# mitake/k8s

Measured on AMD Instinct MI355X. Metric: images/sec ResNet-50 TfJob (train, synthetic ImageNet), higher is better.
Workload: dtype bf16; 1 GPU; model=resnet50-v1.5, global_batch=3072, per_gpu_batch=3072, image_size=224, parallelism=dp1, optimizer=fused SGD momentum 0.9 (HIP)

## Files before the change

### k8s_amd/csrc/binding/conv.cpp

```cpp
#include "binding/common.h"

namespace k8s_amd::binding {
namespace {

int conv_out(int in, int k, int st, int pad, int dil) { return (in + 2 * pad - dil * (k - 1) - 1) / st + 1; }

struct ConvGeom {
  int N, H, W, C, K, R, S;
};
ConvGeom conv_geom(const Tensor& x, const Tensor& w) {
  TORCH_CHECK(x.dim() == 4 && w.dim() == 4, "x [N,H,W,C], w [K,R,S,C]");
  ConvGeom g{(int)x.size(0), (int)x.size(1), (int)x.size(2), (int)x.size(3),
             (int)w.size(0), (int)w.size(1), (int)w.size(2)};
  TORCH_CHECK(w.size(3) == g.C, "channel mismatch");
  TORCH_CHECK(g.C % 8 == 0 && g.K % 8 == 0, "implicit-GEMM conv needs C % 8 == 0 and K % 8 == 0");
  return g;
}
Tensor conv_fwd(Tensor x, Tensor w, int64_t stride, int64_t pad, int64_t dil, bool out_f32, OptTensor bias, int64_t act,
                OptTensor stats, OptTensor xform) {
  check_bf16(x, "x"); check_bf16(w, "w");
  const auto [N, H, W, C, K, R, S] = conv_geom(x, w);
  TORCH_CHECK(stride >= 1 && dil >= 1, "conv_fwd: stride >= 1, dilation >= 1");
  const int Ho = conv_out(H, R, stride, pad, dil), Wo = conv_out(W, S, stride, pad, dil);
  if (bias) check_channel_f32(*bias, K, "bias");
  if (stats) check_stat_sums(*stats, K, "stats", true);
  const float* xf = xform_ptr(xform, C);
  if (xf) TORCH_CHECK(C % 64 == 0 && !out_f32 && !bias && act == 0,
                      "normalize-on-load convolution: C % 64 == 0, bf16 output, no bias / activation");
  auto y = torch::empty({N, Ho, Wo, K}, x.options().dtype(out_f32 ? at::kFloat : at::kBFloat16));
  launch_conv_fwd(cbf(x), cbf(w), y.data_ptr(), out_f32, N, H, W, C, K, R, S, (int)stride, (int)pad, (int)dil, Ho, Wo,
                  optf(bias), (int)act, 0, stats ? f32(*stats) : nullptr, cur_stream(), nullptr, xf);
  return y;
}

Tensor conv_infer(Tensor x, Tensor w, int64_t stride, int64_t pad, Tensor scale, Tensor shift, OptTensor res,
                  bool relu, OptTensor out) {
  check_bf16_dense(x, 4, "x"); check_bf16_dense(w, 4, "w");
  const auto [N, H, W, C, K, R, S] = conv_geom(x, w);
  TORCH_CHECK(stride >= 1 && pad >= 0, "conv_infer: stride >= 1, pad >= 0");
  check_channel_f32(scale, K, "scale"); check_channel_f32(shift, K, "shift");
  TORCH_CHECK(H + 2 * pad >= R && W + 2 * pad >= S, "conv_infer: the filter does not fit the padded image");
  const int Ho = conv_out(H, R, stride, pad, 1), Wo = conv_out(W, S, stride, pad, 1);
  TORCH_CHECK((long)N * Ho * Wo < (1L << 31), "conv_infer: fewer than 2^31 output pixels");
  const std::vector<int64_t> oshape{N, Ho, Wo, K};
  if (out) {
    check_bf16_dense(*out, 4, "out");
    TORCH_CHECK(out->sizes().vec() == oshape, "out must be [N, Ho, Wo, K]");
  }
  if (res) {
    check_bf16_dense(*res, 4, "res");
    TORCH_CHECK(res->sizes().vec() == oshape, "res must have the output's shape [N, Ho, Wo, K]");
  }
  Tensor y = out ? *out : torch::empty(oshape, x.options());
  launch_conv_infer(cbf(x), cbf(w), bf(y), N, H, W, C, K, R, S, (int)stride, (int)pad, Ho, Wo, f32(scale), f32(shift),
                    res ? cbf(*res) : nullptr, relu, cur_stream());
  return y;
}

void conv_fwd_subgrid(Tensor x, Tensor w, int64_t pad, int64_t Hs, int64_t Ws, Tensor out, int64_t stride, int64_t a,
                      int64_t b, bool accumulate, OptTensor bn_x, OptTensor bn_mask, OptTensor bn_mean,
                      OptTensor bn_sums, OptTensor bn_gamma, OptTensor bn_beta, OptTensor bn_invstd) {
  check_bf16(x, "x"); check_bf16(w, "w"); check_bf16(out, "out");
  const auto [N, H, W, C, K, R, S] = conv_geom(x, w);
  TORCH_CHECK(out.dim() == 4 && out.size(0) == N && out.size(3) == K, "out shape");
  const int OH = out.size(1), OW = out.size(2);
  TORCH_CHECK(stride >= 1 && a >= 0 && a < stride && b >= 0 && b < stride, "parity out of range");
  TORCH_CHECK(Hs >= 1 && Ws >= 1 && (Hs - 1) * stride + a < OH && (Ws - 1) * stride + b < OW,
              "sub-grid exceeds the output image");
  k8s_amd::SubGrid sg{OH, OW, (int)stride, (int)a, (int)b};
  k8s_amd::BnBwdSums bb;
  if (bn_sums) {
    TORCH_CHECK(bn_x && bn_mean, "bn sums: bn_x and bn_mean");
    TORCH_CHECK(bn_mask ? accumulate : !accumulate,
                "bn sums: bn_mask + accumulate (a correction) or bn_gamma / bn_beta / bn_invstd + a plain store");
    TORCH_CHECK(bn_x->sizes() == out.sizes(), "bn_x: the shape of out");
    bb = bn_bwd_sums(*bn_x, *bn_mean, *bn_sums, bn_mask, bn_gamma, bn_beta, bn_invstd, {}, {}, {});
  }
  launch_conv_fwd(cbf(x), cbf(w), out.data_ptr(), false, N, H, W, C, K, R, S, 1, (int)pad, 1, (int)Hs, (int)Ws, nullptr,
                  0, accumulate ? 1 : 0, nullptr, cur_stream(), &sg, nullptr, bn_sums ? &bb : nullptr);
}

Tensor conv3x3_dgrad_bnstats(Tensor gy, Tensor wt, Tensor x, Tensor gamma, Tensor beta, Tensor mean, Tensor invstd,
                             Tensor sums) {
  check_bf16_dense(gy, 4, "gy"); check_bf16_dense(wt, 4, "wt"); check_bf16_dense(x, 4, "x");
  const int N = (int)gy.size(0), H = (int)gy.size(1), W = (int)gy.size(2), Kc = (int)gy.size(3);
  const int C = (int)wt.size(0);
  TORCH_CHECK(wt.size(1) == 3 && wt.size(2) == 3 && wt.size(3) == Kc, "wt: [C, 3, 3, K]");
  TORCH_CHECK(x.size(0) == N && x.size(1) == H && x.size(2) == W && x.size(3) == C, "x: the shape of dx");
  TORCH_CHECK(k8s_amd::conv3x3_eligible(H, W, Kc, C, 3, 3, 1, 1, 1), "conv3x3_dgrad_bnstats: outside the kernel");
  const k8s_amd::BnBwdSums bb = bn_bwd_sums(x, mean, sums, {}, gamma, beta, invstd, {}, {}, {});
  Tensor dx = torch::empty({N, H, W, C}, gy.options());
  launch_conv3x3(cbf(gy), cbf(wt), bf(dx), nullptr, nullptr, N, H, W, Kc, C, cur_stream(), &bb);
  return dx;
}

void conv_wgrad(Tensor x, Tensor dy, Tensor dw, int64_t stride, int64_t pad, int64_t dil, int64_t splits,
                bool accumulate, OptTensor xform) {
  check_bf16(x, "x"); check_bf16(dy, "dy");
  check_cuda(dw, "dw"); check_dtype(dw, at::kFloat, "dw");
  const auto [N, H, W, C, K, R, S] = conv_geom(x, dw);
  TORCH_CHECK(stride >= 1 && dil >= 1, "conv_wgrad: stride >= 1, dilation >= 1");
  const int Ho = conv_out(H, R, stride, pad, dil), Wo = conv_out(W, S, stride, pad, dil);
  TORCH_CHECK(dy.dim() == 4 && dy.size(0) == N && dy.size(1) == Ho && dy.size(2) == Wo && dy.size(3) == K,
              "dy shape mismatch");
  const float* xf = xform_ptr(xform, C);
  if (dil == 1 && Ho == H && Wo == W && H == W && k8s_amd::wgrad3x3_tiled_ok(C, K, R, S, (int)stride, (int)pad, W)) {
    auto wsp = torch::empty({k8s_amd::wgrad3x3_tiled_workspace(N, H, W, C)}, dw.options());
    launch_wgrad3x3_tiled(cbf(x), cbf(dy), f32(wsp), f32(dw), N, H, W, C, accumulate, cur_stream(), xf);
    return;
  }
  if (!xf && dil == 1 && k8s_amd::wgrad_stream_eligible(N, Ho, Wo, C, K, R, S)) {
    launch_wgrad_stream(cbf(x), cbf(dy), f32(dw), N, H, W, C, K, R, S, (int)stride, (int)pad, Ho, Wo, accumulate,
                        cur_stream());
    return;
  }
  if (xf) TORCH_CHECK(C % 64 == 0, "normalize-on-load weight gradient needs C % 64 == 0");
  int sp = splits <= 0 ? k8s_amd::gemm_choose_splits(K, R * S * C, N * Ho * Wo) : (int)splits;
  Tensor ws;
  if (sp > 1) ws = torch::empty({k8s_amd::gemm_splitk_workspace(K, R * S * C, sp)}, dw.options());
  launch_conv_wgrad(cbf(x), cbf(dy), f32(dw), N, H, W, C, K, R, S, (int)stride, (int)pad, (int)dil, Ho, Wo, sp,
                    accumulate, sp > 1 ? f32(ws) : nullptr, cur_stream(), xf);
}

std::vector<Tensor> conv_dgrad_wsub(Tensor w, std::vector<std::vector<int64_t>> taps) {
  check_bf16(w, "w");
  TORCH_CHECK(w.dim() == 4, "w [K,R,S,C]");
  const int K = w.size(0), R = w.size(1), S = w.size(2), C = w.size(3);
  TORCH_CHECK(!taps.empty() && taps.size() <= 16, "1-16 parities");
  k8s_amd::DgradTaps t{};
  long off = 0;
  std::vector<int64_t> offs;
  for (size_t p = 0; p < taps.size(); ++p) {
    TORCH_CHECK(!taps[p].empty() && taps[p].size() <= 16, "1-16 taps per parity");
    t.n[p] = (int)taps[p].size();
    t.off[p] = off;
    offs.push_back(off);
    for (size_t i = 0; i < taps[p].size(); ++i) {
      TORCH_CHECK(taps[p][i] >= 0 && taps[p][i] < R * S, "tap index out of range");
      t.rs[p][i] = (int)taps[p][i];
    }
    off += (long)C * t.n[p] * K;
    off = (off + 7) / 8 * 8;
  }
  auto out = torch::empty({off}, w.options());
  launch_conv_dgrad_wsub(cbf(w), bf(out), K, R * S, C, t, (int)taps.size(), cur_stream());
  return {out, torch::tensor(offs)};
}
Tensor conv_dgrad_wtrans(Tensor w) {
  check_bf16(w, "w");
  TORCH_CHECK(w.dim() == 4, "w [K,R,S,C]");
  const int K = w.size(0), R = w.size(1), S = w.size(2), C = w.size(3);
  auto w2 = torch::empty({C, R, S, K}, w.options());
  launch_conv_dgrad_wtrans(cbf(w), bf(w2), K, R, S, C, cur_stream());
  return w2;
}

}

void bind_conv(pybind11::module_& m) {
  m.def("conv_fwd", &conv_fwd, "x"_a, "w"_a, "stride"_a, "pad"_a, "dil"_a, "out_f32"_a, "bias"_a, "act"_a, "stats"_a,
        "xform"_a = py::none());
  m.def("conv_infer", &conv_infer, "x"_a, "w"_a, "stride"_a, "pad"_a, "scale"_a, "shift"_a, "res"_a = py::none(),
        "relu"_a = true, "out"_a = py::none());
  m.def("conv3x3_staged_ok", [](int H, int W, int C, int K, int R, int S, int stride, int pad) {
    return k8s_amd::conv3x3_eligible(H, W, C, K, R, S, stride, pad, 1) &&
           k8s_amd::conv3x3_eligible(H, W, K, C, R, S, stride, pad, 1) &&
           k8s_amd::wgrad3x3_tiled_ok(C, K, R, S, stride, pad, W);
  });
  m.def("conv3x3_dgrad_bnstats", &conv3x3_dgrad_bnstats,
        "3x3 stride-1 data gradient with the BatchNorm-backward sums of a relu(BN(x)) input (conv3x3.hip)");
  m.def("conv_fwd_subgrid", &conv_fwd_subgrid, "x"_a, "w"_a, "pad"_a, "Hs"_a, "Ws"_a, "out"_a, "stride"_a, "a"_a, "b"_a,
        "accumulate"_a = false, "bn_x"_a = py::none(), "bn_mask"_a = py::none(), "bn_mean"_a = py::none(),
        "bn_sums"_a = py::none(), "bn_gamma"_a = py::none(), "bn_beta"_a = py::none(), "bn_invstd"_a = py::none());
  m.def("conv_wgrad", &conv_wgrad, "x"_a, "dy"_a, "dw"_a, "stride"_a, "pad"_a, "dil"_a, "splits"_a, "accumulate"_a,
        "xform"_a = py::none());
  m.def("wgrad_stream_eligible", &k8s_amd::wgrad_stream_eligible, "tall-K weight-gradient kernel takes this shape");
  m.def("conv_dgrad_wtrans", &conv_dgrad_wtrans);
  m.def("conv_dgrad_wsub", &conv_dgrad_wsub);
}

}
```

### k8s_amd/csrc/kernels/launchers.h

```cpp
#pragma once
#include <hip/hip_runtime.h>
#include <stdint.h>

#include "rng.h"

namespace k8s_amd {

int planner_cus();
void set_planner_cus(int n);

void launch_sgd(float* p, float* mom, const void* g, bool g_bf16, uint16_t* pbf, long n, const uint8_t* decay_mask, float lr,
                float mu, float wd, float scale, const float* scale_ptr, const float* hyper, bool nesterov,
                bool first_step, hipStream_t st);
void launch_adam(float* p, float* m1, float* m2, const void* g, bool g_bf16, uint16_t* pbf, long n, const uint8_t* decay_mask,
                 float lr, float b1, float b2, float eps, float wd, float scale, const float* scale_ptr,
                 const float* hyper, float bc1, float bc2, bool decoupled, hipStream_t st);
void launch_sumsq(const void* g, bool g_bf16, long n, float* out, hipStream_t st);
void launch_clip_factor(const float* stats, float max_norm, float* factor, hipStream_t st);
void launch_slice_sum(const uint16_t* in, long n, int world, float* out, uint16_t* out_bf, hipStream_t st);
void launch_cast_bf16(const float* in, uint16_t* out, long n, hipStream_t st);

void launch_grad_accumulate(float* acc, const float* g, long n, bool first, hipStream_t st);
void launch_grad_fold(float* g, const float* acc, uint16_t* out_bf, long n, hipStream_t st);

// ... 20 lines not shown
                             uint16_t* y, const float* sums, int nrep, float* save_mean, float* save_invstd,
                             float* run_mean, float* run_var, float* params, long M, int C, float eps, float momentum,
                             bool relu, hipStream_t st, uint8_t* mask = nullptr, uint16_t* ysub = nullptr,
                             int H = 1, int W = 1);
void launch_bn_fwd_from_sums_dual(const uint16_t* x, const float* gamma, const float* beta, const float* sums,
                                  int nrep, float* save_mean, float* save_invstd, float* run_mean, float* run_var,
                                  float* params, const uint16_t* xr, const float* gamma_r, const float* beta_r,
                                  const float* sums_r, int nrep_r, float* save_mean_r, float* save_invstd_r,
                                  float* run_mean_r, float* run_var_r, float* params_r, uint16_t* y, uint8_t* mask,
                                  long M, int C, float eps, float momentum, hipStream_t st);
void launch_bn_bwd_from_sums(const uint16_t* dy, const uint16_t* x, const uint8_t* mask, const float* sums, int nrep,
                             const float* mean, const float* invstd, const float* gamma, const float* beta,
                             uint16_t* dx, uint16_t* dres, float* dgamma, float* dbeta, float* params, long M, int C,
                             hipStream_t st);
void launch_bn_bwd_relu_from_sums(const uint16_t* dy, const uint16_t* x, const float* sums, int nrep,
                                  const float* mean, const float* invstd, const float* gamma, const float* beta,
                                  uint16_t* dx, float* dgamma, float* dbeta, float* params, long M, int C,
                                  hipStream_t st);
void launch_bn_bwd_dual_from_sums(const uint16_t* dy, const uint8_t* mask, const uint16_t* x, const float* sums,
                                  int nrep, const float* mean, const float* invstd, const float* gamma,
                                  const float* beta, uint16_t* dx, float* dgamma, float* dbeta, float* params,
                                  const uint16_t* x2, const float* sums2, const float* mean2, const float* invstd2,
                                  const float* gamma2, const float* beta2, uint16_t* dx2, float* dgamma2,
                                  float* dbeta2, float* params2, long M, int C, hipStream_t st);
void launch_bn_bwd_dual(const uint16_t* dy, const uint8_t* mask, const uint16_t* x, const float* mean,
                        const float* invstd, const float* gamma, const float* beta, uint16_t* dx, float* dgamma,
                        float* dbeta, float* work, float* params, const uint16_t* x2, const float* mean2,
                        const float* invstd2, const float* gamma2, const float* beta2, uint16_t* dx2, float* dgamma2,
                        float* dbeta2, float* work2, float* params2, long M, int C, hipStream_t st);
void launch_bn_finalize_sums(const float* gamma, const float* beta, const float* sums, int nrep, float* save_mean,
                             float* save_invstd, float* run_mean, float* run_var, float* params, long M, int C,
                             float eps, float momentum, hipStream_t st);
constexpr int kConvStatReplicas = 32;
void launch_bn_bwd(const uint16_t* dy, const uint16_t* x, const float* mean, const float* invstd, const float* gamma,
                   const float* beta, bool relu_x, uint16_t* dx, uint16_t* dres, float* dgamma, float* dbeta,
                   float* work, float* params, long M, int C, hipStream_t st, const uint8_t* mask = nullptr);
void launch_relu_mask(const uint16_t* y, uint8_t* mask, long nvec, hipStream_t st);

void launch_norm_fwd(bool rms, const uint16_t* x, const uint16_t* res, uint16_t* xsum, const float* gamma,
                     const float* beta, uint16_t* y, float* mean, float* rstd, long R, int D, float eps,
                     hipStream_t st, const DropArgs* drop = nullptr);
int norm_workspace_floats(long R, int D);
void launch_norm_bwd(bool rms, const uint16_t* dy, const uint16_t* x, const float* gamma, const float* mean,
                     const float* rstd, const uint16_t* dres, uint16_t* dx, float* dgamma, float* dbeta, float* work,
                     long R, int D, hipStream_t st, float* dsum = nullptr, const DropArgs* drop = nullptr,
                     uint16_t* da = nullptr);

void launch_dropout(const uint16_t* x, uint16_t* y, long R, int D, const DropArgs& dr, hipStream_t st);
void launch_dropout_mask(uint8_t* out, long row0, long R, int C, const DropArgs& dr, hipStream_t st);

void launch_xent_fwd(const void* logits, bool bf16, const int64_t* labels, long R, long V, long ld, float* loss,
                     float* lse, long ignore_index, float smoothing, hipStream_t st);
void launch_xent_bwd(const void* logits, bool bf16, const int64_t* labels, const float* lse, const float* dscale,
                     bool per_row, long R, long V, long ld, void* dlogits, long ignore_index, float smoothing,
                     hipStream_t st);
void launch_xent_eval(const void* logits, bool bf16, const int64_t* labels, long R, long V, long ld, float* loss,
                      int* rank, long ignore_index, hipStream_t st);

int gemm_choose_splits(int M, int N, int K);
struct AddEpi {
  const uint16_t* src;
  const uint8_t* mask;
};
bool gemm_short_ok(int M, int N, int K, long lda, long ldc);
bool gemm_short_bnstats_ok(int M, int N, int K, bool dual);
struct BnBwdSums {
  const uint16_t* x = nullptr;
  const float* gamma = nullptr;
  const float* beta = nullptr;
  const float* mean = nullptr;
  const float* invstd = nullptr;
  float* sums = nullptr;
  const uint8_t* mask = nullptr;
  const uint16_t* x2 = nullptr;
  const float* mean2 = nullptr;
  float* sums2 = nullptr;
};
struct GemmShortBnStats {
  const uint16_t* x = nullptr;
  const uint8_t* mask = nullptr;
  const float* mean = nullptr;
  float* sums = nullptr;
  const uint16_t* x2 = nullptr;
  const float* mean2 = nullptr;
  float* sums2 = nullptr;
};
void launch_gemm_short(const uint16_t* A, const uint16_t* B, long ldb, bool b_mn, uint16_t* C, const uint16_t* add,
                       const uint8_t* mask, const float* xf, float* stats, int M, int N, int K, int epi,
                       hipStream_t st, const GemmShortBnStats* bst = nullptr);
void launch_gemm_dgrad_bnstats(const uint16_t* A, const uint16_t* B, uint16_t* C, int M, int N, int K,
                               const BnBwdSums& bb, hipStream_t st, bool accumulate = false,
                               const uint16_t* add_src = nullptr, const uint8_t* add_mask = nullptr);
void launch_gemm(const uint16_t* A, long lda, bool a_kmajor, const uint16_t* B, long ldb, bool b_kmajor, void* C,
                 long ldc, bool c_f32, int M, int N, int K, const float* bias, int act, uint16_t* pre, int mode,
                 float alpha, int splits, float* ws, hipStream_t st, const AddEpi* add = nullptr,
                 const float* xform_b = nullptr, int xform_c = 0);
void launch_mask_apply(const uint16_t* src, const uint8_t* mask, uint16_t* out, long n, hipStream_t st);
long gemm_splitk_workspace(int M, int N, int splits);
bool conv3x3_eligible(int H, int W, int C, int K, int R, int S, int stride, int pad, int dil);
void launch_conv3x3(const uint16_t* x, const uint16_t* w, uint16_t* y, float* stats, const float* xform, int N,
                    int H, int W, int C, int K, hipStream_t st,
                    const BnBwdSums* bsums = nullptr);
bool gemm256_eligible(int M, int N, int K, bool a_kmajor, bool b_kmajor);
int gemm256_choose_splits(int M, int N, int K);
bool gemm_w4_dact_ok(int M, int N, int K, long lda, long ldb, long ldc);
long gemm_w4_dact_part_floats(int M, int N);
void launch_gemm_w4_dact(const uint16_t* A, long lda, const uint16_t* B, long ldb, uint16_t* C, long ldc, int M, int N,
                         int K, const uint16_t* pre, int act, float* part, float* db, bool db_accumulate,
                         float* sk_slabs, int* sk_sync, hipStream_t st);
bool gemm_w4_swiglu_ok(int M, int F, int K, long lda, long ldb);
void launch_gemm_w4_swiglu_bwd(const uint16_t* A, long lda, const uint16_t* B, long ldb, uint16_t* dgu,
                               const uint16_t* gu, int M, int F, int K, int blk, float* sk_slabs, int* sk_sync,
                               hipStream_t st);
bool gemm_w4_stats_ok(int M, int N, int K);
bool gemm_w4_dgrad_bnstats_ok(int M, int N, int K);
void launch_gemm_w4_dgrad_bnstats(const uint16_t* A, const uint16_t* B, uint16_t* y, int M, int N, int K,
                                  const uint16_t* x, const float* tab, float* sums, float* sk_slabs, int* sk_sync,
                                  hipStream_t st);
void launch_gemm_w4_stats(const uint16_t* A, long lda, const uint16_t* B, long ldb, uint16_t* y, int M, int N, int K,
                          float* stats, float* sk_slabs, int* sk_sync, hipStream_t st);
bool gemm_w4_rope_ok(int M, int N, int K, long lda, long ldb, int rot_cols);
void launch_gemm_w4_rope(const uint16_t* A, long lda, const uint16_t* B, long ldb, uint16_t* y, int M, int N, int K,
                         const int* pos, const float* table, int rot_cols, float* sk_slabs, int* sk_sync,
                         hipStream_t st);
bool gemm_w4_swiglu_fwd_ok(int M, int F, int K, long lda, long ldb);
void launch_gemm_w4_swiglu_fwd(const uint16_t* A, long lda, const uint16_t* B, long ldb, uint16_t* gu, uint16_t* h,
                               int M, int F, int K, float* sk_slabs, int* sk_sync, hipStream_t st);
struct Gemm256Plan {
  int tiles, full, sk, kps;
};
Gemm256Plan gemm256_plan(int M, int N, int K);
long gemm256_sk_slab_floats(const Gemm256Plan& p);
long gemm256_sk_sync_ints(const Gemm256Plan& p);
void launch_gemm256(const uint16_t* A, long lda, bool a_kmajor, const uint16_t* B, long ldb, bool b_kmajor, void* C,
                    long ldc, bool c_f32, int M, int N, int K, const float* bias, int act, uint16_t* pre,
                    bool accumulate, float alpha, hipStream_t st, int splits = 1, float* ws = nullptr,
                    float* sk_slabs = nullptr, int* sk_sync = nullptr);
struct SubGrid {
  int H, W, stride, a, b;
};
void launch_conv_fwd(const uint16_t* x, const uint16_t* w, void* y, bool y_f32, int N, int H, int W, int C, int K,
                     int R, int S, int stride, int pad, int dil, int Ho, int Wo, const float* bias, int act,
                     int mode, float* stats, hipStream_t st, const SubGrid* sg = nullptr, const float* xform = nullptr,
                     const BnBwdSums* bb = nullptr);
void launch_conv_infer(const uint16_t* x, const uint16_t* w, uint16_t* y, int N, int H, int W, int C, int K, int R,
                       int S, int stride, int pad, int Ho, int Wo, const float* scale, const float* shift,
                       const uint16_t* res, bool relu, hipStream_t st);
void launch_conv_wgrad(const uint16_t* x, const uint16_t* dy, float* dw, int N, int H, int W, int C, int K, int R,
                       int S, int stride, int pad, int dil, int Ho, int Wo, int splits, bool accumulate, float* ws,
                       hipStream_t st, const float* xform = nullptr);
bool wgrad_stream_eligible(int N, int Ho, int Wo, int C, int K, int R, int S);
void launch_wgrad_stream(const uint16_t* x, const uint16_t* dy, float* dw, int N, int H, int W, int C, int K, int R,
                         int S, int stride, int pad, int Ho, int Wo, bool accumulate, hipStream_t st);
void launch_conv_dgrad_wtrans(const uint16_t* w, uint16_t* w2, int K, int R, int S, int C, hipStream_t st);
struct DgradTaps {
  int n[16];
  long off[16];
  int rs[16][16];
};
void launch_conv_dgrad_wsub(const uint16_t* w, uint16_t* out, int K, int RS, int C, const DgradTaps& taps, int np,
                            hipStream_t st);

void launch_swiglu_fwd(const uint16_t* gu, uint16_t* y, long T, int F, int blk, hipStream_t st);
void launch_swiglu_bwd(const uint16_t* gu, const uint16_t* dy, uint16_t* dgu, long T, int F, int blk, hipStream_t st);
void launch_rope(uint16_t* x, long ld, const int* pos, const float* table, long T, int H, int D, bool inverse,
                 hipStream_t st);
void launch_gelu_bwd(const uint16_t* dy, const uint16_t* pre, uint16_t* dx, long n, hipStream_t st);
void launch_relu_bwd(const uint16_t* dy, const uint16_t* y, uint16_t* dx, long n, hipStream_t st);
int colsum_workspace_floats(long R, int C);
void launch_colsum(const uint16_t* x, long R, int C, float* work, float* out, bool accumulate, hipStream_t st);
void launch_colsum_fold(float* part, int P, int C, float* out, bool accumulate, hipStream_t st);
void launch_colsum_group(float* part, int P, int C, int gs, hipStream_t st);
void launch_act_bwd_colsum(int act, const uint16_t* dy, const uint16_t* pre, uint16_t* g, long R, int C, float* work,
                           float* out, bool accumulate, hipStream_t st);

struct AttnFwdArgs {
  const uint16_t *q, *k, *v;
  uint16_t* o;
  float* lse;
  const int* kv_lens;
  long sqb, sqs, sqh, skb, sks, skh, svb, svs, svh, sob, sos, soh;
  long lse_ld;
  int B, Sq, Sk, Hq, Hkv, causal;
  float scale_log2;
  DropArgs drop;
};
struct AttnBwdArgs {
  const uint16_t *q, *k, *v, *dO;
  const float* lse;
  float* delta;
  uint16_t* dq;
  uint16_t *dk, *dv;
  const int* kv_lens;
  long sqb, sqs, sqh, skb, sks, skh, svb, svs, svh, sdb, sds, sdh;
  long sgqb, sgqs, sgqh, sgkb, sgks, sgkh, sgvb, sgvs, sgvh;
  long lse_ld;
  int B, Sq, Sk, Hq, Hkv, causal;
  float scale_log2, scale;
  int dkv_split = 1;
  float* dkv_ws = nullptr;
  float* cpart = nullptr;
  int cpart_ld = 0;
  DropArgs drop;
};
int flash_dkv_splits(int B, int Sq, int Sk, int Hkv, int causal);
bool flash_bwd_one_block(int D, int Sq, int Sk, int Hq, int Hkv, int dkv_split);
void launch_bn_relu_maxpool_fwd(const uint16_t* x, const float* gamma, const float* beta, const float* sums, int nrep,
                                float* save_mean, float* save_invstd, float* run_mean, float* run_var, float* params,
                                uint16_t* y, uint8_t* idx, int N, int H, int W, int C, float eps, float momentum,
                                hipStream_t st, uint16_t* xarg = nullptr, uint8_t* ybits = nullptr);
void launch_pool_bn_bwd_from_sums(const uint16_t* dpool, const uint8_t* idx, const uint16_t* x, const float* mean,
                                  const float* invstd, const float* gamma, const float* beta, uint16_t* dx,
                                  float* dgamma, float* dbeta, const float* sums, int nrep, float* params, int N,
                                  int H, int W, int C, hipStream_t st);
int pool_bn_workspace_floats(int C);
void launch_pool_bn_bwd(const uint16_t* dpool, const uint8_t* idx, const uint16_t* x, const float* mean,
                        const float* invstd, const float* gamma, const float* beta, uint16_t* dx, float* dgamma,
                        float* dbeta, float* work, float* params, int N, int H, int W, int C, hipStream_t st);

int stream_order_mode();
int stream_dir(int fixed);

void launch_flash_fwd(const AttnFwdArgs& a, int D, hipStream_t st);
void launch_flash_bwd(const AttnBwdArgs& a, int D, const uint16_t* o, long sob, long sos, long soh, hipStream_t st);

struct EmbTable {
  const uint16_t* w;
  float* g;
  const int64_t* ids;
  int V;
};
void launch_embed_fwd(const EmbTable* tabs, int ntab, int T, int D, int S, uint16_t* out, hipStream_t st);
void launch_embed_bwd(const EmbTable* tabs, int ntab, int T, int D, int S, const uint16_t* g, hipStream_t st);

void launch_avgpool_fwd(const uint16_t* x, uint16_t* y, int N, int HW, int C, hipStream_t st);
void launch_avgpool_bwd(const uint16_t* dy, uint16_t* dx, int N, int HW, int C, hipStream_t st);

void launch_stem_s2d_input(const uint16_t* x, int N, int H, int W, int Cin, int pad, uint16_t* out, hipStream_t st);
void launch_stem_w_s2d(const uint16_t* w7, int K, int R, int Cw, uint16_t* w4, hipStream_t st);
bool stem_conv_fwd_ok(int K, int R, int C, int Wo);
void launch_stem_conv_fwd(const uint16_t* xs, const uint16_t* w4, uint16_t* y, float* stats, int N, int Hs, int Ws,
                          hipStream_t st);
void splitk_reduce(const float* ws, int splits, long mn, float* out, bool accumulate, hipStream_t st);
bool wgrad3x3_tiled_ok(int C, int K, int R, int S, int stride, int pad, int W);
int wgrad3x3_tiled_blocks(int N, int H, int W, int C);
long wgrad3x3_tiled_workspace(int N, int H, int W, int C);
void launch_wgrad3x3_tiled(const uint16_t* x, const uint16_t* dy, float* ws, float* dw, int N, int H, int W, int C,
                           bool accumulate, hipStream_t st, const float* xform = nullptr);
int stem_wgrad_blocks(int N, int Hs);
void launch_stem_wgrad(const uint16_t* xs, const uint16_t* dy, float* ws, float* dw4, int N, int Hs, int Ws,
                       hipStream_t st);
void launch_stem_dw_s2d(const float* dw4, int K, int R, int Cw, float* dw7, hipStream_t st);

void launch_subsample_nhwc(const uint16_t* x, uint16_t* y, int N, int H, int W, int C, int s, hipStream_t st);
void launch_maxpool_fwd(const uint16_t* x, uint16_t* y, uint8_t* idx, int N, int H, int W, int C, int Ho, int Wo,
                        int k, int s, int p, hipStream_t st);
void launch_maxpool_bwd(const uint16_t* dy, const uint8_t* idx, uint16_t* dx, int N, int H, int W, int C, int Ho,
                        int Wo, int k, int s, int p, hipStream_t st);

}
```

### k8s_amd/ops/conv.py

```python
from __future__ import annotations

import os
import warnings

import torch
import torch.nn.functional as F

from k8s_amd.ops._ext import load as _load



STATS = {"hip_fwd": 0, "aten_fwd": 0, "hip_wgrad": 0, "aten_wgrad": 0, "hip_dgrad": 0, "aten_dgrad": 0,
         "bn_bstats": 0, "hip_infer": 0, "aten_infer": 0}



def _nchw(x):
    return x.permute(0, 3, 1, 2)


def _nhwc(y):
    return y.permute(0, 2, 3, 1).contiguous()


# ... 80 lines not shown
BSTATS_STRIDED = os.environ.get("K8S_AMD_BN_BSTATS_STRIDED", "0") != "0"
BSTATS_TILE_SHORT = os.environ.get("K8S_AMD_BN_BSTATS_TILE_SHORT", "0") != "0"


def _bn_sums(C_, bn_link, C, device):
    R = C_.conv_stat_replicas
    if bn_link.store is not None:
        from k8s_amd.ops.nn import _zero_scratch
        return _zero_scratch(bn_link.store, device, R * 2 * C).view(R, 2, C)
    return torch.zeros(R, 2, C, device=device, dtype=torch.float32)


def _dgrad_hip(C_, gy, w, padding, addend=None, bn_link=None):
    K, R, S, C = w.shape
    masked = addend is not None and not torch.is_tensor(addend)
    if (BSTATS_3X3 and bn_link is not None and bn_link.relu and bn_link.x is not None and addend is None and R == 3
            and S == 3
            and padding == 1 and gy.shape[1] == gy.shape[2] and bn_link.x.shape[:3] == gy.shape[:3]
            and C_.conv3x3_staged_ok(gy.shape[1], gy.shape[2], C, K, 3, 3, 1, 1)):
        sums = _bn_sums(C_, bn_link, C, gy.device)
        dx = C_.conv3x3_dgrad_bnstats(gy, C_.conv_dgrad_wtrans(w), bn_link.x, bn_link.gamma, bn_link.beta,
                                      bn_link.mean, bn_link.invstd, sums)
        bn_link.deposit(sums, None, dx)
        return dx
    if R == 1 and S == 1 and padding == 0:
        N, H, W_, _ = gy.shape
        if masked and bn_link is not None and not bn_link.relu and bn_link.x is not None and \
                bn_link.x.shape == (N, H, W_, C) and \
                C_.gemm_short_bnstats_ok(N * H * W_, C, K, bn_link.x2 is not None):
            sums = _bn_sums(C_, bn_link, C, gy.device)
            sums2 = _bn_sums(C_, bn_link, C, gy.device) if bn_link.x2 is not None else None
            out = C_.dgrad_short_bnstats(
                gy.reshape(-1, K), w.reshape(K, C), addend.dy.view(-1, C), addend.mask, bn_link.x.view(-1, C),
                bn_link.mask, bn_link.mean, sums, None if sums2 is None else bn_link.x2.view(-1, C), bn_link.mean2,
                sums2).view(N, H, W_, C)
            bn_link.deposit(sums, sums2, out)
            return out
        if (masked and BSTATS_TILE_MASK and bn_link is not None and not bn_link.relu and bn_link.x is not None
                and bn_link.mask is not None and bn_link.x.shape == (N, H, W_, C) and N * H * W_ < 2 ** 31
                and (BSTATS_TILE_SHORT or bn_link.x2 is None or not C_.gemm_short_bnstats_ok(N * H * W_, C, K, False))):
            out = torch.empty(N, H, W_, C, device=gy.device, dtype=gy.dtype)
            sums = _bn_sums(C_, bn_link, C, gy.device)
            dual = bn_link.x2 is not None
            sums2 = _bn_sums(C_, bn_link, C, gy.device) if dual else None
            C_.gemm_dgrad_bnstats_mask(gy.reshape(-1, K), w.reshape(K, C), out.view(-1, C), bn_link.x.view(-1, C),
                                       bn_link.mask, bn_link.mean, sums, addend.dy.view(-1, C), addend.mask,
                                       bn_link.x2.view(-1, C) if dual else None, bn_link.mean2 if dual else None,
                                       sums2)
            bn_link.deposit(sums, sums2, out)
            return out
        if (BSTATS_GEMM and bn_link is not None and bn_link.relu and bn_link.x is not None and addend is None
                and bn_link.x.shape == (N, H, W_, C) and C_.gemm_dgrad_bnstats_ok(N * H * W_, C, K)):
            sums = _bn_sums(C_, bn_link, C, gy.device)
            out = C_.gemm_dgrad_bnstats(gy.reshape(-1, K), w.reshape(K, C), bn_link.x.view(-1, C), bn_link.gamma,
                                        bn_link.beta, bn_link.mean, bn_link.invstd, sums).view(N, H, W_, C)
            bn_link.deposit(sums, None, out)
            return out
        if (BSTATS_ENTRY and addend is None and bn_link is not None and not bn_link.relu and not bn_link.last_full and bn_link.mask is not None
                and bn_link.x2 is None and bn_link.x is not None and bn_link.x.shape == (N, H, W_, C)
                and C_.gemm_short_bnstats_ok(N * H * W_, C, K, False)):
            sums = _bn_sums(C_, bn_link, C, gy.device)
            out = C_.dgrad_short_bnstats(gy.reshape(-1, K), w.reshape(K, C), None, None, bn_link.x.view(-1, C),
                                         bn_link.mask, bn_link.mean, sums).view(N, H, W_, C)
            bn_link.deposit_pending(sums)
            return out
        if masked:
            out = torch.empty(N, H, W_, C, device=gy.device, dtype=gy.dtype)
            C_.gemm(gy.reshape(-1, K), True, w.reshape(K, C), False, out.view(-1, C), False, None, 0, None, True,
                    1.0, 1, add_src=addend.dy.view(-1, C), add_mask=addend.mask)
            return out
        if (addend is not None and bn_link is not None and bn_link.last_full and bn_link.x is not None
                and bn_link.mask is not None and bn_link.x.shape == (N, H, W_, C) and addend.is_contiguous()
                and C % 8 == 0 and N * H * W_ < 2 ** 31):
            sums = _bn_sums(C_, bn_link, C, gy.device)
            C_.gemm_dgrad_bnstats_mask(gy.reshape(-1, K), w.reshape(K, C), addend.view(-1, C), bn_link.x.view(-1, C),
                                       bn_link.mask, bn_link.mean, sums)
            bn_link.deposit(sums, None, addend)
            return addend
        if addend is not None:
            C_.gemm(gy.reshape(-1, K), True, w.reshape(K, C), False, addend.view(-1, C), False, None, 0, None, True,
                    1.0, 1)
            return addend
        return C_.gemm(gy.reshape(-1, K), True, w.reshape(K, C), False, None, False, None, 0, None, False, 1.0,
                       1).reshape(N, H, W_, C)
    if masked:
        addend = addend.materialize()
    dx = C_.conv_fwd(gy, C_.conv_dgrad_wtrans(w), 1, R - 1 - padding, 1, False, None, 0, None)
    return dx if addend is None else dx.add_(addend)


def _parity_taps(R, a, pad, stride):
    taps = sorted(((a + pad - r) // stride, r) for r in range(R) if (a + pad - r) % stride == 0)
    if taps and [d for d, _ in taps] != list(range(taps[0][0], taps[0][0] + len(taps))):
        return None
    return taps


def strided_dgrad_ok(gy, w, stride, padding):
    K, R, S, C = w.shape
    if stride < 2 or K % 8 or C % 8:
        return False
    for a in range(stride):
        for b in range(stride):
            tr, ts = _parity_taps(R, a, padding, stride), _parity_taps(S, b, padding, stride)
            if tr is None or ts is None:
                return False
            if tr and ts and tr[0][0] != ts[0][0]:
                return False
    return True


def _dgrad_strided_hip(C_, gy, w, stride, padding, H, W, addend=None, bn_link=None):
    K, R, S, C = w.shape
    N = gy.shape[0]
    fix = (bn_link is not None and bn_link.pending and R == 1 and S == 1 and padding == 0 and addend is not None
           and torch.is_tensor(addend) and addend.is_contiguous() and bn_link.x is not None
           and bn_link.x.shape == addend.shape)
    if bn_link is not None and bn_link.pending and not fix:
        bn_link.sums, bn_link.pending = None, False
    relu_sums = (BSTATS_STRIDED and bn_link is not None and bn_link.relu and bn_link.x is not None and addend is None
                 and not bn_link.pending and bn_link.x.shape == (N, H, W, C) and C > 64 and K % 64 == 0)
    rsums = _bn_sums(C_, bn_link, C, gy.device) if relu_sums else None
    parities = [(a, b) for a in range(stride) for b in range(stride)]
    empty = [(a, b) for a, b in parities
             if not _parity_taps(R, a, padding, stride) or not _parity_taps(S, b, padding, stride)]
    if addend is not None:
        dx = addend
    else:
        dx = (torch.zeros if empty else torch.empty)(N, H, W, C, device=gy.device, dtype=gy.dtype)
    live = [(a, b, _parity_taps(R, a, padding, stride), _parity_taps(S, b, padding, stride))
            for a in range(stride) for b in range(stride)]
    live = [(a, b, tr, ts) for a, b, tr, ts in live if tr and ts]
    packed, offs = C_.conv_dgrad_wsub(w, [[r * S + s_ for _, r in tr for _, s_ in ts] for _, _, tr, ts in live])
    offs = offs.tolist()
    for i, (a, b, tr, ts) in enumerate(live):
        n = C * len(tr) * len(ts) * K
        wsub = packed[offs[i]:offs[i] + n].view(C, len(tr), len(ts), K)
        Hs, Ws = (H - a + stride - 1) // stride, (W - b + stride - 1) // stride
        if fix:
            C_.conv_fwd_subgrid(gy, wsub, -tr[0][0], Hs, Ws, dx, stride, a, b, True, bn_link.x, bn_link.mask,
                                bn_link.mean, bn_link.sums)
        elif relu_sums:
            C_.conv_fwd_subgrid(gy, wsub, -tr[0][0], Hs, Ws, dx, stride, a, b, False, bn_link.x, None, bn_link.mean,
                                rsums, bn_link.gamma, bn_link.beta, bn_link.invstd)
        else:
            C_.conv_fwd_subgrid(gy, wsub, -tr[0][0], Hs, Ws, dx, stride, a, b, addend is not None)
    if fix:
        bn_link.complete(dx)
    if relu_sums:
        bn_link.deposit(rsums, None, dx)
    return dx


def conv_bwd(gy, x, w, stride, padding, need_dx, p=None, addend=None, xform=None, x_sub=None, bn_link=None):
    K, R, S, C = w.shape
    C_ = _load() if gy.is_cuda else None
    if x_sub is not None:
        _wgrad_hip(C_, gy, x_sub, p.grad.view(p.shape), 1, 0, p.written)
        STATS["hip_wgrad"] += 1
        p.store._notify(p) if p.written else p.store.mark_written(p)
        p = None
    hip = _hip(gy, x, w)
    if xform is not None and not (hip and C % 64 == 0 and K % 8 == 0 and p is not None
                                  and p.grad.dtype == torch.float32):
        raise RuntimeError("normalize-on-load weight gradient outside the kernels' contract")
    if addend is not None and not torch.is_tensor(addend) and not (
            hip and stride == 1 and K % 8 == 0 and C % 8 == 0):
        addend = addend.materialize()
    dw_done = False
    if hip and C % 8 == 0 and K % 8 == 0 and p is not None and p.grad.dtype == torch.float32:
        STATS["hip_wgrad"] += 1
        acc = p.written
        _wgrad_hip(C_, gy, x, p.grad.view(p.shape), stride, padding, acc, xform)
        if acc:
            p.store._notify(p)
        else:
            p.store.mark_written(p)
        dw_done = True
    dx = None
    if need_dx:
        if hip and stride == 1 and K % 8 == 0 and C % 8 == 0:
            STATS["hip_dgrad"] += 1
            dx = _dgrad_hip(C_, gy, w, padding, addend, bn_link)
        elif hip and strided_dgrad_ok(gy, w, stride, padding):
            STATS["hip_dgrad"] += 1
            dx = _dgrad_strided_hip(C_, gy, w, stride, padding, x.shape[1], x.shape[2], addend, bn_link)
        else:
            _vendor("dgrad", x, w, stride, padding)
            dx, _ = _aten_bwd(gy, x, w, stride, padding, True, False)
            if addend is not None:
                dx = dx + addend
    return _finish_dw(dx, dw_done, p, gy, x, w, stride, padding)


SUB1X1 = os.environ.get("K8S_AMD_SUB1X1", "1") != "0"


def subsample_ok(x, w, stride, padding) -> bool:
    K, R, S, C = w.shape
    return (SUB1X1 and stride > 1 and R == 1 and S == 1 and padding == 0 and _hip(x, w) and C % 64 == 0
            and K % 8 == 0 and x.is_contiguous())


def _finish_dw(dx, dw_done, p, gy, x, w, stride, padding):
    if not dw_done and p is not None:
        _vendor("wgrad", x, w, stride, padding)
        _, dw = _aten_bwd(gy, x, w, stride, padding, False, True)
        p.store.deposit(p, dw)
    return dx
```

Baseline: 15680 images/s.

## Fuse 1x1 conv backward dgrad, wgrad and BatchNorm-backward sums into one kernel

Adds a HIP kernel for the bottleneck 1x1 expansion convs (C,K = 64,256 or 128,512). In one persistent pass over row tiles it computes the data gradient with MFMA and writes it out. It also applies the BN normalize-on-load to x to build the weight gradient, and accumulates the BN-backward sums for the upstream relu(BN) input. This avoids reading gy and x several times across separate dgrad, wgrad and stats kernels. The cost is heavy register and LDS use at one block per CU, plus atomic dw and sums reductions. The path is on by default behind an env flag.

```diff
diff --git a/k8s_amd/csrc/binding/conv.cpp b/k8s_amd/csrc/binding/conv.cpp
--- a/k8s_amd/csrc/binding/conv.cpp
+++ b/k8s_amd/csrc/binding/conv.cpp
@@ -92,6 +92,23 @@
   Tensor dx = torch::empty({N, H, W, C}, gy.options());
   launch_conv3x3(cbf(gy), cbf(wt), bf(dx), nullptr, nullptr, N, H, W, Kc, C, cur_stream(), &bb);
   return dx;
+}
+
+Tensor bwd1x1_fused(Tensor gy, Tensor x, Tensor w, Tensor xform, Tensor gamma, Tensor beta, Tensor mean, Tensor invstd,
+                    Tensor dw, Tensor sums, bool accumulate) {
+  check_bf16_dense(gy, 2, "gy"); check_bf16_dense(x, 2, "x"); check_bf16_dense(w, 2, "w");
+  const long M = gy.size(0), K = gy.size(1), C = x.size(1);
+  TORCH_CHECK(x.size(0) == M && w.size(0) == K && w.size(1) == C, "shapes: gy [M, K], x [M, C], w [K, C]");
+  TORCH_CHECK(k8s_amd::bwd1x1_fused_ok(M, (int)C, (int)K),
+              "bwd1x1_fused: (C, K) = (64, 256) or (128, 512), 1 <= M < 2^31");
+  check_cuda(dw, "dw"); check_dtype(dw, at::kFloat, "dw"); check_aligned(dw, "dw");
+  TORCH_CHECK(dw.numel() == K * C, "dw must have K * C fp32 elements");
+  check_channel_f32(xform, 2 * C, "xform (BatchNorm scale | shift)");
+  const k8s_amd::BnBwdSums bb = bn_bwd_sums(x, mean, sums, {}, gamma, beta, invstd, {}, {}, {});
+  Tensor dz = torch::empty({M, C}, gy.options());
+  launch_bwd1x1_fused(cbf(gy), cbf(x), cbf(w), f32(xform), bb.gamma, bb.beta, bb.mean, bb.invstd, bf(dz), f32(dw),
+                      bb.sums, M, (int)C, (int)K, accumulate, cur_stream());
+  return dz;
 }
 
 void conv_wgrad(Tensor x, Tensor dy, Tensor dw, int64_t stride, int64_t pad, int64_t dil, int64_t splits,
@@ -174,7 +191,13 @@
         "bn_sums"_a = py::none(), "bn_gamma"_a = py::none(), "bn_beta"_a = py::none(), "bn_invstd"_a = py::none());
   m.def("conv_wgrad", &conv_wgrad, "x"_a, "dy"_a, "dw"_a, "stride"_a, "pad"_a, "dil"_a, "splits"_a, "accumulate"_a,
         "xform"_a = py::none());
-  m.def("wgrad_stream_eligible", &k8s_amd::wgrad_stream_eligible, "tall-K weight-gradient kernel takes this shape");
+  m.def("bwd1x1_fused", &bwd1x1_fused, "gy"_a, "x"_a, "w"_a, "xform"_a, "gamma"_a, "beta"_a, "mean"_a, "invstd"_a,
+        "dw"_a, "sums"_a, "accumulate"_a,
+        "1x1 data gradient, normalize-on-load weight gradient and BatchNorm-backward sums in one pass (bwd1x1_fused.hip)");
+  m.def("bwd1x1_fused_ok", [](int64_t M, int64_t C, int64_t K) {
+    return C <= 1024 && K <= 4096 && k8s_amd::bwd1x1_fused_ok(M, (int)C, (int)K);
+  }, "M"_a, "C"_a, "K"_a, "whether bwd1x1_fused takes this shape");
+  m.def("wgrad_stream_eligible",&k8s_amd::wgrad_stream_eligible, "tall-K weight-gradient kernel takes this shape");
   m.def("conv_dgrad_wtrans", &conv_dgrad_wtrans);
   m.def("conv_dgrad_wsub", &conv_dgrad_wsub);
 }
diff --git a/k8s_amd/csrc/kernels/bwd1x1_fused.hip b/k8s_amd/csrc/kernels/bwd1x1_fused.hip
--- /dev/null
+++ b/k8s_amd/csrc/kernels/bwd1x1_fused.hip
@@ -0,0 +1,309 @@
+#include <algorithm>
+#include <stdexcept>
+
+#include "common.h"
+#include "launchers.h"
+#include "mfma.h"
+
+namespace k8s_amd {
+namespace b1f {
+
+constexpr int THREADS = 512;
+constexpr int CT = 64;
+
+__device__ __attribute__((aligned(64))) uint16_t g_zero16[64];
+
+typedef __attribute__((ext_vector_type(4))) int int4_t;
+
+__device__ __forceinline__ int swz128(int r) { return 2 * (((r >> 1) & 1) | (((r >> 3) & 1) << 1)); }
+__device__ __forceinline__ int swz_g(int r) { return (2 * ((r & 3) | (((r >> 3) & 1) << 2))) | ((r >> 2) & 1); }
+
+struct TrRaw {
+  short4_t lo, hi;
+};
+template <int RB, bool G>
+__device__ __forceinline__ void tr_load(TrRaw& r, const char* img, int rb, int kk, int lane) {
+  const int g = lane >> 4, i = lane & 15, q = i >> 2, p = i & 3;
+  const int u = (rb >> 3) + (p >> 1);
+  const int r0 = kk * 32 + 8 * g + q, r1 = r0 + 4;
+  const int u0 = u ^ (G ? swz_g(r0) : swz128(r0)), u1 = u ^ (G ? swz_g(r1) : swz128(r1));
+  tr16_asm(r.lo, img + r0 * RB + (u0 << 4) + (p & 1) * 8);
+  tr16_asm(r.hi, img + r1 * RB + (u1 << 4) + (p & 1) * 8);
+}
+#define K8S_LDS_TIE4(w, a, b, c, d) asm volatile(w : "+v"(a), "+v"(b), "+v"(c), "+v"(d))
+
+struct Args {
+  const uint16_t *gy, *x, *w;
+  const float *xform, *gamma, *beta, *mean, *invstd;
+  uint16_t* dz;
+  float* dw;
+  float* sums;
+  int M, C, ntiles, npairs;
+};
+
+__device__ __forceinline__ void lds_barrier() {
+  asm volatile("s_waitcnt lgkmcnt(0)" ::: "memory");
+  __builtin_amdgcn_s_barrier();
+  asm volatile("" ::: "memory");
+}
+
+template <int K, int RS, int NSLOT, int HALVES>
+__global__ void __launch_bounds__(THREADS, 1) bwd1x1_fused_kernel(Args a) {
+  constexpr int RB = K * 2, UG = K / 8;
+  constexpr int IMG_G = RS * RB, IMG_X = RS * 128, STAGE = IMG_G + IMG_X, RING = NSLOT * STAGE;
+  constexpr int LG = RS * UG / THREADS;
+  constexpr int XT = RS * 8;
+  constexpr int NKS = K / 32, KW = K / 8, KTW = KW / 16;
+  static_assert(LG * THREADS == RS * UG && XT % 64 == 0 && XT <= THREADS && (RS == 32 || RS == 64), "tile");
+  static_assert(XT * 64 <= RING, "sums partials reuse the ring");
+  constexpr bool PLDS = K > 256;
+  __shared__ __attribute__((aligned(1024))) char smem[RING + IMG_X + (PLDS ? 5 * CT * 4 : 0)];
+  char* stg = smem + RING;
+  float* ptab = reinterpret_cast<float*>(stg + IMG_X);
+
+  const int tid = threadIdx.x, lane = tid & 63;
+  const int wid = __builtin_amdgcn_readfirstlane(tid >> 6);
+  const int bid = blockIdx.x;
+  int pair = bid, chalf = 0;
+  if constexpr (HALVES == 2) {
+    const int slot = bid >> 3;
+    chalf = slot & 1;
+    pair = (slot >> 1) * 8 + (bid & 7);
+  }
+  const int c0 = chalf * CT;
+  const int n = pair < a.ntiles ? (a.ntiles - pair + a.npairs - 1) / a.npairs : 0;
+  if (n == 0) return;
+  const long M = a.M;
+  const int C = a.C;
+
+  const int ct = wid & 3, rh = wid >> 2;
+  int4_t wf[NKS];
+  {
+    const uint16_t* wp = a.w + (long)(8 * (lane >> 4)) * C + c0 + ct * 16 + (lane & 15);
+#pragma unroll
+    for (int ks = 0; ks < NKS; ++ks) {
+      bf16x8_t v;
+#pragma unroll
+      for (int j = 0; j < 8; ++j) v[j] = (short)wp[(long)(ks * 32 + j) * C];
+      wf[ks] = __builtin_bit_cast(int4_t, v);
+    }
+  }
+  const int erow = tid >> 3;
+  const int eu = (tid & 7) ^ swz128(erow);
+  const int ecol = c0 + eu * 8;
+  float xsc[8], xsh[8], gsc[8], gsh[8], mu[8], ps[8], pq[8];
+#pragma unroll
+  for (int j = 0; j < 8; ++j) {
+    xsc[j] = a.xform[ecol + j];
+    xsh[j] = a.xform[C + ecol + j];
+    mu[j] = a.mean[ecol + j];
+    bn_affine_regs(a.gamma[ecol + j], a.beta[ecol + j], mu[j], a.invstd[ecol + j], gsc[j], gsh[j]);
+    ps[j] = pq[j] = 0.f;
+  }
+  if constexpr (PLDS) {
+    if (tid < 8) {
+#pragma unroll
+      for (int j = 0; j < 8; ++j) {
+        ptab[0 * CT + tid * 8 + j] = xsc[j];
+        ptab[1 * CT + tid * 8 + j] = xsh[j];
+        ptab[2 * CT + tid * 8 + j] = gsc[j];
+        ptab[3 * CT + tid * 8 + j] = gsh[j];
+        ptab[4 * CT + tid * 8 + j] = mu[j];
+      }
+    }
+  }
+#pragma unroll
+  for (int ks = 0; ks < NKS; ++ks) asm volatile("" : "+v"(wf[ks]));
+  if constexpr (!PLDS) {
+#pragma unroll
+    for (int j = 0; j < 8; ++j) asm volatile("" : "+v"(xsc[j]), "+v"(xsh[j]), "+v"(gsc[j]), "+v"(gsh[j]), "+v"(mu[j]));
+  } else {
+    __syncthreads();
+  }
+
+  auto issue = [&](int slot, int i) {
+    char* st = smem + slot * STAGE;
+    const long m0 = (long)(pair + i * a.npairs) * RS;
+#pragma unroll
+    for (int j = 0; j < LG; ++j) {
+      const int sl = j * THREADS + tid, row = sl / UG, up = sl % UG;
+      const int u = up ^ swz_g(row);
+      const long m = m0 + row;
+      const void* src = m < M ? (const void*)(a.gy + m * K + u * 8) : (const void*)g_zero16;
+      glds16(src, st + j * (THREADS * 16) + wid * 1024);
+    }
+    if (wid < XT / 64) {
+      const long m = m0 + erow;
+      const void* src = m < M ? (const void*)(a.x + m * C + ecol) : (const void*)g_zero16;
+      glds16(src, st + IMG_G + wid * 1024);
+    }
+  };
+
+  f32x4_t dwa[KTW][4];
+#pragma unroll
+  for (int i = 0; i < KTW; ++i)
+#pragma unroll
+    for (int j = 0; j < 4; ++j) dwa[i][j] = f32x4_t{0.f, 0.f, 0.f, 0.f};
+
+  const int pre = min(n, NSLOT - 1);
+  for (int s = 0; s < pre; ++s) issue(s, s);
+  int slot = 0;
+  for (int s = 0; s < n; ++s) {
+    const int younger = min(n - 1, s + NSLOT - 2) - s;
+    if (younger >= 2) asm volatile("s_waitcnt vmcnt(%0)" ::"n"(2 * LG) : "memory");
+    else if (younger == 1) asm volatile("s_waitcnt vmcnt(%0)" ::"n"(LG) : "memory");
+    else asm volatile("s_waitcnt vmcnt(0)" ::: "memory");
+    lds_barrier();
+    if (s + NSLOT - 1 < n) issue(slot == 0 ? NSLOT - 1 : slot - 1, s + NSLOT - 1);
+    char* G = smem + slot * STAGE;
+    char* X = G + IMG_G;
+
+    {
+      f32x4_t d0 = {0.f, 0.f, 0.f, 0.f}, d1 = {0.f, 0.f, 0.f, 0.f};
+      const int row0 = rh * (RS / 2) + (lane & 15);
+      const int kq = lane >> 4;
+      if constexpr (RS == 64) {
+        const int row1 = row0 + 16;
+        const char* p0 = G + row0 * RB;
+        const char* p1 = G + row1 * RB;
+        const int s0 = swz_g(row0), s1 = swz_g(row1);
+#pragma unroll
+        for (int ks = 0; ks < NKS; ++ks) {
+          const bf16x8_t b0 = *reinterpret_cast<const bf16x8_t*>(p0 + (((ks * 4 + kq) ^ s0) << 4));
+          const bf16x8_t b1 = *reinterpret_cast<const bf16x8_t*>(p1 + (((ks * 4 + kq) ^ s1) << 4));
+          const mfma_bf16x8 wa = __builtin_bit_cast(mfma_bf16x8, wf[ks]);
+          d0 = mfma16(wa, __builtin_bit_cast(mfma_bf16x8, b0), d0);
+          d1 = mfma16(wa, __builtin_bit_cast(mfma_bf16x8, b1), d1);
+        }
+      } else {
+        const char* p0 = G + row0 * RB;
+        const int s0 = swz_g(row0);
+#pragma unroll
+        for (int ks = 0; ks < NKS; ks += 2) {
+          const bf16x8_t b0 = *reinterpret_cast<const bf16x8_t*>(p0 + (((ks * 4 + kq) ^ s0) << 4));
+          const bf16x8_t b1 = *reinterpret_cast<const bf16x8_t*>(p0 + (((ks * 4 + 4 + kq) ^ s0) << 4));
+          d0 = mfma16(__builtin_bit_cast(mfma_bf16x8, wf[ks]), __builtin_bit_cast(mfma_bf16x8, b0), d0);
+          d1 = mfma16(__builtin_bit_cast(mfma_bf16x8, wf[ks + 1]), __builtin_bit_cast(mfma_bf16x8, b1), d1);
+        }
+        d0 += d1;
+      }
+      const int unit = ct * 2 + (lane >> 5), half = (lane >> 4) & 1;
+      auto put = [&](int row, const f32x4_t& d) {
+        bf16x4_t o;
+#pragma unroll
+        for (int r = 0; r < 4; ++r) o[r] = (short)f2bf(d[r]);
+        *reinterpret_cast<bf16x4_t*>(stg + row * 128 + ((unit ^ swz128(row)) << 4) + half * 8) = o;
+      };
+      put(row0, d0);
+      if constexpr (RS == 64) put(row0 + 16, d1);
+    }
+    lds_barrier();
+
+    if (wid < XT / 64) {
+      const bf16x8_t dzv = *reinterpret_cast<const bf16x8_t*>(stg + tid * 16);
+      const bf16x8_t xv = *reinterpret_cast<const bf16x8_t*>(X + tid * 16);
+      if constexpr (PLDS) {
+        const float* t = ptab + (ecol - c0);
+#pragma unroll
+        for (int j = 0; j < 8; ++j) {
+          xsc[j] = t[j];
+          xsh[j] = t[CT + j];
+          gsc[j] = t[2 * CT + j];
+          gsh[j] = t[3 * CT + j];
+          mu[j] = t[4 * CT + j];
+        }
+      }
+      float o[8];
+#pragma unroll
+      for (int j = 0; j < 8; ++j) {
+        const float xf = bf2f((uint16_t)xv[j]);
+        o[j] = fmaxf(__builtin_fmaf(xf, xsc[j], xsh[j]), 0.f);
+        const float g = relu_on(xf, gsc[j], gsh[j]) ? bf2f((uint16_t)dzv[j]) : 0.f;
+        ps[j] += g;
+        pq[j] = __builtin_fmaf(g, xf - mu[j], pq[j]);
+      }
+      *reinterpret_cast<bf16x8_t*>(X + tid * 16) = pack_bf16x8(o);
+      const long m = (long)(pair + s * a.npairs) * RS + erow;
+      if (m < M) *reinterpret_cast<bf16x8_t*>(a.dz + m * C + ecol) = dzv;
+    }
+    lds_barrier();
+
+#pragma unroll
+    for (int kk = 0; kk < RS / 32; ++kk) {
+      TrRaw ar[KTW], br[4];
+#pragma unroll
+      for (int j = 0; j < 4; ++j) tr_load<128, false>(br[j], X, j * 16, kk, lane);
+#pragma unroll
+      for (int i = 0; i < KTW; ++i) tr_load<RB, true>(ar[i], G, wid * KW + i * 16, kk, lane);
+      K8S_LDS_TIE8("s_waitcnt lgkmcnt(0)", br[0].lo, br[0].hi, br[1].lo, br[1].hi, br[2].lo, br[2].hi, br[3].lo,
+                   br[3].hi);
+#pragma unroll
+      for (int i = 0; i < KTW; i += 2)
+        K8S_LDS_TIE4("s_waitcnt lgkmcnt(0)", ar[i].lo, ar[i].hi, ar[i + 1].lo, ar[i + 1].hi);
+#pragma unroll
+      for (int i = 0; i < KTW; ++i)
+#pragma unroll
+        for (int j = 0; j < 4; ++j)
+          dwa[i][j] = __builtin_amdgcn_mfma_f32_16x16x32_bf16(join8(br[j].lo, br[j].hi), join8(ar[i].lo, ar[i].hi),
+                                                              dwa[i][j], 0, 0, 0);
+    }
+    slot = slot + 1 == NSLOT ? 0 : slot + 1;
+  }
+
+#pragma unroll
+  for (int i = 0; i < KTW; ++i) {
+    const int k = wid * KW + i * 16 + (lane & 15);
+#pragma unroll
+    for (int j = 0; j < 4; ++j) {
+      float* d = a.dw + (long)k * C + c0 + j * 16 + 4 * (lane >> 4);
+#pragma unroll
+      for (int r = 0; r < 4; ++r) atomicAdd(d + r, dwa[i][j][r]);
+    }
+  }
+  __syncthreads();
+  float* part = reinterpret_cast<float*>(smem);
+  if (tid < XT) {
+#pragma unroll
+    for (int j = 0; j < 8; ++j) {
+      part[tid * 16 + j] = ps[j];
+      part[tid * 16 + 8 + j] = pq[j];
+    }
+  }
+  __syncthreads();
+  if (tid < 2 * CT) {
+    const int col = tid & (CT - 1), which = tid / CT;
+    const int u = col >> 3, r = col & 7;
+    float v = 0.f;
+#pragma unroll 4
+    for (int row = 0; row < RS; ++row) v += part[(row * 8 + (u ^ swz128(row))) * 16 + which * 8 + r];
+    atomicAdd(a.sums + (long)(bid % kConvStatReplicas) * 2 * C + (long)which * C + c0 + col, v);
+  }
+}
+
+}
+
+bool bwd1x1_fused_ok(long M, int C, int K) {
+  return M >= 1 && M < (1L << 31) && ((C == 64 && K == 256) || (C == 128 && K == 512));
+}
+
+void launch_bwd1x1_fused(const uint16_t* gy, const uint16_t* x, const uint16_t* w, const float* xform,
+                         const float* gamma, const float* beta, const float* mean, const float* invstd, uint16_t* dz,
+                         float* dw, float* sums, long M, int C, int K, bool accumulate, hipStream_t st) {
+  using namespace b1f;
+  if (!bwd1x1_fused_ok(M, C, K)) throw std::runtime_error("bwd1x1_fused: (C, K) = (64, 256) or (128, 512), M < 2^31");
+  if (!accumulate) (void)hipMemsetAsync(dw, 0, (size_t)K * C * sizeof(float), st);
+  Args a{gy, x, w, xform, gamma, beta, mean, invstd, dz, dw, sums, (int)M, C, 0, 0};
+  const int cus = std::max(1, planner_cus());
+  if (C == 64) {
+    a.ntiles = (int)((M + 63) / 64);
+    a.npairs = cus;
+    hipLaunchKernelGGL((bwd1x1_fused_kernel<256, 64, 3, 1>), dim3(cus), dim3(THREADS), 0, st, a);
+  } else {
+    const int grid = std::max(16, cus / 16 * 16);
+    a.ntiles = (int)((M + 31) / 32);
+    a.npairs = grid / 2;
+    hipLaunchKernelGGL((bwd1x1_fused_kernel<512, 32, 4, 2>), dim3(grid), dim3(THREADS), 0, st, a);
+  }
+}
+
+}
diff --git a/k8s_amd/csrc/kernels/launchers.h b/k8s_amd/csrc/kernels/launchers.h
--- a/k8s_amd/csrc/kernels/launchers.h
+++ b/k8s_amd/csrc/kernels/launchers.h
@@ -196,6 +196,10 @@
 bool wgrad_stream_eligible(int N, int Ho, int Wo, int C, int K, int R, int S);
 void launch_wgrad_stream(const uint16_t* x, const uint16_t* dy, float* dw, int N, int H, int W, int C, int K, int R,
                          int S, int stride, int pad, int Ho, int Wo, bool accumulate, hipStream_t st);
+bool bwd1x1_fused_ok(long M, int C, int K);
+void launch_bwd1x1_fused(const uint16_t* gy, const uint16_t* x, const uint16_t* w, const float* xform,
+                         const float* gamma, const float* beta, const float* mean, const float* invstd, uint16_t* dz,
+                         float* dw, float* sums, long M, int C, int K, bool accumulate, hipStream_t st);
 void launch_conv_dgrad_wtrans(const uint16_t* w, uint16_t* w2, int K, int R, int S, int C, hipStream_t st);
 struct DgradTaps {
   int n[16];
diff --git a/k8s_amd/ops/conv.py b/k8s_amd/ops/conv.py
--- a/k8s_amd/ops/conv.py
+++ b/k8s_amd/ops/conv.py
@@ -256,6 +256,16 @@
     return dx
 
 
+def _bwd1x1_fused_on() -> bool:
+    return os.environ.get("K8S_AMD_BWD1X1_FUSED", "1") != "0"
+
+
+def _fused_link_ok(bn_link, x) -> bool:
+    return (bn_link is not None and bn_link.relu and bn_link.x is not None and bn_link.x.shape == x.shape
+            and bn_link.x.data_ptr() == x.data_ptr()
+            and all(t is not None for t in (bn_link.gamma, bn_link.beta, bn_link.mean, bn_link.invstd)))
+
+
 def conv_bwd(gy, x, w, stride, padding, need_dx, p=None, addend=None, xform=None, x_sub=None, bn_link=None):
     K, R, S, C = w.shape
     C_ = _load() if gy.is_cuda else None
@@ -271,6 +281,21 @@
     if addend is not None and not torch.is_tensor(addend) and not (
             hip and stride == 1 and K % 8 == 0 and C % 8 == 0):
         addend = addend.materialize()
+    if (xform is not None and need_dx and addend is None and R == 1 and S == 1 and stride == 1 and padding == 0
+            and _bwd1x1_fused_on() and _fused_link_ok(bn_link, x) and gy.is_contiguous() and x.is_contiguous()
+            and C_.bwd1x1_fused_ok(gy.numel() // K, C, K)):
+        STATS["hip_wgrad"] += 1
+        STATS["hip_dgrad"] += 1
+        acc = p.written
+        sums = _bn_sums(C_, bn_link, C, gy.device)
+        dz = C_.bwd1x1_fused(gy.view(-1, K), x.view(-1, C), w.view(K, C), xform, bn_link.gamma, bn_link.beta,
+                             bn_link.mean, bn_link.invstd, p.grad.view(K, C), sums, acc).view(x.shape)
+        if acc:
+            p.store._notify(p)
+        else:
+            p.store.mark_written(p)
+        bn_link.deposit(sums, None, dz)
+        return dz
     dw_done = False
     if hip and C % 8 == 0 and K % 8 == 0 and p is not None and p.grad.dtype == torch.float32:
         STATS["hip_wgrad"] += 1
```

After: 16200 images/s (median of 6 runs). +3.3%, better.
